# chalharu/rust-compression

Measured on AMD Instinct MI355X. Metric: BZip2 level-9 encode MB/s (input bytes, HBM-resident in and out: the kernels' rate; value_end_to_end is host buffer to host buffer at the C ABI), higher is better.
Workload: dtype u8/u32

## Files before the change

### rust-compression_amd/csrc/k_mtf.hip

```cpp
#include "bzgpu.h"
#include <cstdlib>

namespace bzgpu {

constexpr u32 kChunkWGs = (kMaxMtfChunks + 255) / 256;
constexpr u32 kMtfSmallAlpha = 96;

__device__ __forceinline__ u32 popc8(const u32 *b)
{
    u32 c = 0;
#pragma unroll
    for (int i = 0; i < 8; ++i) c += __popc(b[i]);
    return c;
}

__device__ __forceinline__ u32 block_excl_sum(u32 v, u32 *sh , u32 &total)
{
    const u32 l = lane_id(), w = threadIdx.x >> 6;
    const u32 inc = wave_incl_sum(v);
    if (l == 63) sh[w] = inc;
    __syncthreads();
    u32 carry = 0, tot = 0;
    for (u32 k = 0; k < kSortThreads / 64; ++k) {
        if (k < w) carry += sh[k];
        tot += sh[k];
    }
    total = tot;
    __syncthreads();
    return carry + inc - v;
}

constexpr u32 kMtfDense = 0x80000000u;
__device__ __forceinline__ bool mtf_collapsed(const MtfArgs &a, u32 lb) { return a.heads && !(a.hcount[lb] & kMtfDense); }
__device__ __forceinline__ u32 mtf_len(const MtfArgs &a, u32 lb) { return mtf_collapsed(a, lb) ? a.hcount[lb] : a.blocks[lb].n; }
__device__ __forceinline__ const u8 *mtf_seq(const MtfArgs &a, u32 lb) { return (mtf_collapsed(a, lb) ? a.H : a.L) + (size_t)lb * kSlot; }

__global__ __launch_bounds__(kSortThreads) void k_mtf_heads_mark(MtfArgs a)
{
    __shared__ u32 s_cnt[kSortThreads / 64];
    const u32 lb = blockIdx.y, tile = blockIdx.x;
    const u32 n = a.blocks[lb].n;
    if (n == 0u && tile == 0u && threadIdx.x == 0u) a.hcount[lb] = 0u;
    if (tile * kSortTile >= n) return;
    const u8 *L = a.L + (size_t)lb * kSlot;
    const u32 p0 = tile * kSortTile + threadIdx.x * 16u;
    const u32 valid = p0 < n ? ((n - p0) < 16u ? (n - p0) : 16u) : 0u;
    u32 hb = 0;
    if (valid) {
        const uint4 q = *reinterpret_cast<const uint4 *>(L + p0);
        const u32 prev = p0 ? (u32)L[p0 - 1u] : 0u;
        const u32 wv[4] = {q.x, q.y, q.z, q.w};
        u32 carry = prev;
#pragma unroll
        for (u32 w = 0; w < 4; ++w) {
            const u32 d = wv[w] ^ ((wv[w] << 8) | carry);
            carry = wv[w] >> 24;
#pragma unroll
            for (u32 k = 0; k < 4; ++k) hb |= ((d >> (8u * k)) & 0xFFu) ? (1u << (4u * w + k)) : 0u;
        }
        if (p0 == 0u) hb |= 1u;
        hb &= 0xFFFFu >> (16u - valid);
        a.headbits[(((size_t)lb * kSlot) >> 4) + (p0 >> 4)] = (u16)hb;
    }
    const u32 c = wave_sum((u32)__popc(hb));
    if (lane_id() == 0) s_cnt[threadIdx.x >> 6] = c;
    __syncthreads();
    if (threadIdx.x == 0) {
        u32 t = 0;
        for (u32 k = 0; k < kSortThreads / 64; ++k) t += s_cnt[k];
        a.tile_hcnt[lb * kTilesPerBlock + tile] = t;
    }
}

__global__ __launch_bounds__(kSortThreads) void k_mtf_heads_pack(MtfArgs a)
{
    __shared__ __attribute__((aligned(16))) u8 s_h[kSortTile + 16];
    __shared__ u32 s_su[kSortThreads / 64];
    __shared__ u32 s_pre[4];
    const u32 lb = blockIdx.y, tile = blockIdx.x;
    const u32 n = a.blocks[lb].n;
    if (tile * kSortTile >= n) return;
    const u8 *L = a.L + (size_t)lb * kSlot;
    const u32 p0 = tile * kSortTile + threadIdx.x * 16u;
    const bool valid = p0 < n;
    if (threadIdx.x < 128u) {
        static_assert(kTilesPerBlock <= 128, "two waves sum the tiles in front");
        const u32 ntiles = (n + kSortTile - 1u) / kSortTile;
        const u32 c = threadIdx.x < ntiles ? a.tile_hcnt[lb * kTilesPerBlock + threadIdx.x] : 0u;
        const u32 pre = wave_sum(threadIdx.x < tile ? c : 0u), all = wave_sum(c);
        if (lane_id() == 0) {
            s_pre[threadIdx.x >> 6] = pre;
            s_pre[2u + (threadIdx.x >> 6)] = all;
        }
    }
    __syncthreads();
    const u32 m = s_pre[2] + s_pre[3];
    if ((u64)m * 1000u > (u64)n * a.dense_permille) {
        if (tile == 0u && threadIdx.x == 0u) a.hcount[lb] = kMtfDense | m;
        return;
    }
    const u32 hb = valid ? (u32)a.headbits[(((size_t)lb * kSlot) >> 4) + (p0 >> 4)] : 0u;
    const uint4 q = valid ? *reinterpret_cast<const uint4 *>(L + p0) : make_uint4(0, 0, 0, 0);
    u32 total;
    const u32 excl = block_excl_sum((u32)__popc(hb), s_su, total);
    const u32 base = s_pre[0] + s_pre[1];
    const u32 al = base & 3u;
    {
        const u32 wv[4] = {q.x, q.y, q.z, q.w};
        u32 pos = al + excl;
#pragma unroll
        for (u32 k = 0; k < 16; ++k)
            if ((hb >> k) & 1u) s_h[pos++] = (u8)(wv[k >> 2] >> ((k & 3) * 8));
    }
    __syncthreads();
    u8 *dst = a.H + (size_t)lb * kSlot + (base - al);
    const u32 endb = al + total;
    for (u32 j = threadIdx.x; j * 4u < endb; j += kSortThreads) {
        if (j * 4u >= al && j * 4u + 4u <= endb) {
            reinterpret_cast<u32 *>(dst)[j] = reinterpret_cast<const u32 *>(s_h)[j];
        } else {
            for (u32 b = j * 4u; b < j * 4u + 4u; ++b)
                if (b >= al && b < endb) dst[b] = s_h[b];
        }
    }
    if (threadIdx.x == 0) {
        a.tile_hbase[lb * kTilesPerBlock + tile] = base;
        if (tile == 0u) a.hcount[lb] = m;
    }
}

__global__ __launch_bounds__(256) void k_mtf_summaries(MtfArgs a)
{
    __shared__ u32 s_seen[8 * 256];
    const u32 lb = blockIdx.y;
    const u32 n = mtf_len(a, lb);
    const u32 chunk = blockIdx.x * 256u + threadIdx.x;
    const u32 beg = chunk * kMtfChunk;
    if (beg >= n) return;
    const u32 end = (beg + kMtfChunk < n) ? beg + kMtfChunk : n;
    const u32 alpha = popc8(a.inuse_bits + lb * 8);
#pragma unroll
    for (int i = 0; i < 8; ++i) s_seen[i * 256 + threadIdx.x] = 0;
    const u8 *L = mtf_seq(a, lb);
    u8 *out = a.summ + ((size_t)lb * kMaxMtfChunks + chunk) * 256u;
    u32 cnt = 0;
    for (int v4 = (int)(kMtfChunk / 64u) - 1; v4 >= 0 && cnt < alpha; --v4) {
        if (beg + (u32)v4 * 64u >= end) continue;
        uint4 q4[4];
#pragma unroll
        for (int u = 0; u < 4; ++u) {
            const u32 pl = beg + (u32)v4 * 64u + (u32)u * 16u;
            q4[u] = (pl < end) ? *reinterpret_cast<const uint4 *>(L + pl) : make_uint4(0, 0, 0, 0);
        }
#pragma unroll
        for (int u = 3; u >= 0; --u) {
            const u32 p0 = beg + (u32)v4 * 64u + (u32)u * 16u;
            if (p0 >= end || cnt >= alpha) continue;
            const u32 wv[4] = {q4[u].x, q4[u].y, q4[u].z, q4[u].w};
#pragma unroll
            for (int k = 15; k >= 0; --k) {
                if (p0 + (u32)k < end) {
                    const u32 c = (wv[k >> 2] >> ((k & 3) * 8)) & 0xFFu;
                    const u32 bit = 1u << (c & 31u);
                    const u32 wd = s_seen[(c >> 5) * 256 + threadIdx.x];
                    if (!(wd & bit)) {
                        s_seen[(c >> 5) * 256 + threadIdx.x] = wd | bit;
                        out[cnt++] = (u8)c;
                    }
                }
            }
        }
    }
    a.summ_len[(size_t)lb * kMaxMtfChunks + chunk] = (u16)cnt;
}


constexpr u32 kMtfGroup = 32;
constexpr u32 kMtfGroups = (kMaxMtfChunks + kMtfGroup - 1) / kMtfGroup;

__device__ __forceinline__ u32 mtf_apply_report(u8 *s_list, u32 len, u32 m, u32 w, u8 *s_new, u8 *s_mark, u32 l)
{
    reinterpret_cast<u32 *>(s_mark)[l] = 0;
    __syncthreads();
#pragma unroll
    for (u32 k = 0; k < 4; ++k) {
        const u32 i = l * 4u + k;
        if (i < m) {
            const u8 v = (u8)(w >> (8u * k));
            s_mark[v] = 1;
            s_new[i] = v;
        }
    }
    __syncthreads();
    u32 keep[4], nk = 0;
    u8 ev[4];
#pragma unroll
    for (u32 k = 0; k < 4; ++k) {
        const u32 e = l * 4 + k;
        ev[k] = s_list[e];
        keep[k] = (e < len && !s_mark[ev[k]]) ? 1u : 0u;
        nk += keep[k];
    }
    const u32 inc = wave_incl_sum(nk);
    u32 pos = m + inc - nk;
#pragma unroll
    for (u32 k = 0; k < 4; ++k)
        if (keep[k]) s_new[pos++] = ev[k];
    const u32 kept = __shfl(inc, 63, 64);
    __syncthreads();
    reinterpret_cast<u32 *>(s_list)[l] = reinterpret_cast<u32 *>(s_new)[l];
    __syncthreads();
    return m + kept;
}

__global__ __launch_bounds__(64) void k_mtf_merge_groups(MtfArgs a)
{
    __shared__ u8 s_cur[256], s_new[256], s_mark[256];
    const u32 lb = blockIdx.y, l = threadIdx.x;
    const u32 n = mtf_len(a, lb);
    const u32 nchunks = (n + kMtfChunk - 1) / kMtfChunk;
    const u32 c0 = blockIdx.x * kMtfGroup;
    if (c0 + 2u > nchunks) return;
    const size_t rep0 = (size_t)lb * kMaxMtfChunks;
    const bool act = l * 4u < popc8(a.inuse_bits + lb * 8);
    u32 len = a.summ_len[rep0 + c0];
    reinterpret_cast<u32 *>(s_cur)[l] = act ? reinterpret_cast<const u32 *>(a.summ + (rep0 + c0) * 256u)[l] : 0u;
    __syncthreads();
    u32 c1 = c0 + kMtfGroup;
    if (c1 > nchunks - 1u) c1 = nchunks - 1u;
    u32 m_next = c0 + 1u < c1 ? (u32)a.summ_len[rep0 + c0 + 1u] : 0u;
    u32 w_next = (c0 + 1u < c1 && act) ? reinterpret_cast<const u32 *>(a.summ + (rep0 + c0 + 1u) * 256u)[l] : 0u;
    for (u32 c = c0 + 1u; c < c1; ++c) {
        const u32 m = m_next, w = w_next;
        if (c + 1u < c1) {
            m_next = a.summ_len[rep0 + c + 1u];
            w_next = act ? reinterpret_cast<const u32 *>(a.summ + (rep0 + c + 1u) * 256u)[l] : 0u;
        }
        len = mtf_apply_report(s_cur, len, m, w, s_new, s_mark, l);
        if (act) reinterpret_cast<u32 *>(a.summ + (rep0 + c) * 256u)[l] = reinterpret_cast<u32 *>(s_cur)[l];
        if (l == 0) a.summ_len[rep0 + c] = (u16)len;
    }
}

__global__ __launch_bounds__(64) void k_mtf_group_starts(MtfArgs a)
{
    __shared__ u8 s_state[256], s_new[256], s_mark[256];
    const u32 lb = blockIdx.x, l = threadIdx.x;
    const u32 n = mtf_len(a, lb);
    const u32 nchunks = (n + kMtfChunk - 1) / kMtfChunk;
    const u32 *bits = a.inuse_bits + lb * 8;
    {
        u32 before = 0;
        for (u32 q = 0; q < (l * 4u) / 32u; ++q) before += __popc(bits[q]);
        const u32 wd = bits[(l * 4u) >> 5];
        const u32 sh = (l * 4u) & 31u;
        before += __popc(wd & ((1u << sh) - 1u));
        reinterpret_cast<u32 *>(s_state)[l] = 0;
        __syncthreads();
        u32 pos = before;
        for (u32 k = 0; k < 4; ++k)
            if ((wd >> (sh + k)) & 1u) s_state[pos++] = (u8)(l * 4u + k);
    }
    __syncthreads();
    const u32 alpha = popc8(bits);
    const size_t rep0 = (size_t)lb * kMaxMtfChunks;
    const bool act = l * 4u < alpha;
    for (u32 c0 = 0; c0 < nchunks; c0 += kMtfGroup) {
        if (act) reinterpret_cast<u32 *>(a.init_state + (rep0 + c0) * 256u)[l] = reinterpret_cast<u32 *>(s_state)[l];
        if (c0 + 2u > nchunks) break;
        u32 e = c0 + kMtfGroup - 1u;
        if (e > nchunks - 2u) e = nchunks - 2u;
        const u32 m = a.summ_len[rep0 + e];
        const u32 w = act ? reinterpret_cast<const u32 *>(a.summ + (rep0 + e) * 256u)[l] : 0u;
        (void)mtf_apply_report(s_state, alpha, m, w, s_new, s_mark, l);
    }
}

__global__ __launch_bounds__(256) void k_mtf_chunk_starts(MtfArgs a)
{
    __shared__ u8 s_state[4][256], s_new[4][256], s_mark[4][256];
    const u32 lb = blockIdx.y, l = threadIdx.x & 63u, wv = threadIdx.x >> 6;
    const u32 n = mtf_len(a, lb);
    const u32 nchunks = (n + kMtfChunk - 1) / kMtfChunk;
    const u32 c0 = blockIdx.x * kMtfGroup;
    if (c0 + 1u >= nchunks) return;
    const u32 alpha = popc8(a.inuse_bits + lb * 8);
    const size_t rep0 = (size_t)lb * kMaxMtfChunks;
    const bool act = l * 4u < alpha;
    const u32 g32 = act ? reinterpret_cast<const u32 *>(a.init_state + (rep0 + c0) * 256u)[l] : 0u;
    for (u32 k = 0; k < kMtfGroup / 4u; ++k) {
        const u32 c = c0 + 1u + k * 4u + wv;
        const bool live = c < nchunks && c < c0 + kMtfGroup;
        reinterpret_cast<u32 *>(s_state[wv])[l] = g32;
        const u32 m = live ? (u32)a.summ_len[rep0 + c - 1u] : 0u;
        const u32 w = (live && act) ? reinterpret_cast<const u32 *>(a.summ + (rep0 + c - 1u) * 256u)[l] : 0u;
        (void)mtf_apply_report(s_state[wv], alpha, m, w, s_new[wv], s_mark[wv], l);
        if (live && act) reinterpret_cast<u32 *>(a.init_state + (rep0 + c) * 256u)[l] = reinterpret_cast<u32 *>(s_state[wv])[l];
    }
}


constexpr u32 kMtfSmallPairs = kMtfSmallAlpha / 2;
constexpr u32 kMtfSubBlocks = 16;
typedef short short2_t __attribute__((ext_vector_type(2)));
__device__ __forceinline__ short2_t as_short2(u32 v)
{
    short2_t r;
    __builtin_memcpy(&r, &v, 4);
    return r;
}
template <u32 PAIRS, u32 LANES, u32 ALPHA_LO, u32 SUB = 1>
__global__ __launch_bounds__(LANES) void k_mtf_ranks_small(MtfArgs a)
{
    constexpr u32 CL = LANES / SUB;
    __shared__ u32 s_last[PAIRS * CL];
    __shared__ u8 s_code[256];
    const u32 lb = blockIdx.y;
    const u32 n = mtf_len(a, lb);
    const u32 chunk0 = blockIdx.x * CL;
    const u32 sub = threadIdx.x % SUB;
    if (chunk0 * kMtfChunk >= n) return;
    const u32 *bits = a.inuse_bits + lb * 8;
    const u32 alpha = popc8(bits);
    if (alpha > 2u * PAIRS || alpha <= ALPHA_LO) return;
    for (u32 v = threadIdx.x; v < 256u; v += LANES) {
        u32 before = 0;
        for (u32 q = 0; q < (v >> 5); ++q) before += __popc(bits[q]);
        before += __popc(bits[v >> 5] & ((1u << (v & 31u)) - 1u));
        s_code[v] = (u8)before;
    }
    __syncthreads();
    const u32 chunk = chunk0 + threadIdx.x / SUB;
    const u32 beg = chunk * kMtfChunk;
    if (beg >= n) return;
    const u32 end = (beg + kMtfChunk < n) ? beg + kMtfChunk : n;
    const u32 npairs = (alpha + 1u) >> 1;
    u32 *my = s_last + threadIdx.x / SUB;
    constexpr u32 kPB = 32;
    static_assert(PAIRS % (2u * kPB) == 0 || PAIRS <= kMtfSmallPairs, "the compare loop takes the table two blocks at a time");
    const u32 npairs16 = ((npairs + 2u * kPB - 1u) / (2u * kPB) * (2u * kPB)) < PAIRS ? ((npairs + 2u * kPB - 1u) / (2u * kPB) * (2u * kPB)) : PAIRS;
    for (u32 q = sub; q < (SUB > 1 ? PAIRS : npairs16); q += SUB) my[q * CL] = 0x80008000u;
    if (SUB > 1) {
        __builtin_amdgcn_fence(__ATOMIC_ACQ_REL, "workgroup");
        __builtin_amdgcn_wave_barrier();
    }
    if (sub == 0) {
        const u8 *st = a.init_state + ((size_t)lb * kMaxMtfChunks + chunk) * 256u;
        for (u32 q = 0; q < alpha; ++q) {
            const u32 c = s_code[st[q]];
            const u32 t = (u32)(0xFFFFu - q) & 0xFFFFu;
            u32 wd = my[(c >> 1) * CL];
            wd = (c & 1u) ? ((wd & 0x0000FFFFu) | (t << 16)) : ((wd & 0xFFFF0000u) | t);
            my[(c >> 1) * CL] = wd;
        }
    }
    if (SUB > 1) {
        __builtin_amdgcn_fence(__ATOMIC_ACQ_REL, "workgroup");
        __builtin_amdgcn_wave_barrier();
    }
    const u8 *L = mtf_seq(a, lb);
    u8 *R8 = a.rank8 + (size_t)lb * kSlot;
    for (u32 v4 = 0; v4 < kMtfChunk / 64u; ++v4) {
        if (beg + v4 * 64u >= end) break;
        uint4 q4[4];
#pragma unroll
        for (u32 u = 0; u < 4; ++u) {
            const u32 pl = beg + v4 * 64u + u * 16u;
            q4[u] = (pl < end) ? *reinterpret_cast<const uint4 *>(L + pl) : make_uint4(0, 0, 0, 0);
        }
#pragma unroll
      for (u32 u = 0; u < 4; ++u) {
        const u32 v = v4 * 4u + u;
        const u32 p0 = beg + v * 16u;
        if (p0 >= end) break;
        const u32 wv[4] = {q4[u].x, q4[u].y, q4[u].z, q4[u].w};
        u32 ov[4] = {0, 0, 0, 0};
#pragma unroll
        for (u32 k = 0; k < 16; ++k) {
            u32 rank = 0;
            if (p0 + k < end) {
                const u32 c = s_code[(wv[k >> 2] >> ((k & 3) * 8)) & 0xFFu];
                const u32 wc = my[(c >> 1) * CL];
                const u32 lsu = (c & 1u) ? (wc >> 16) : (wc & 0xFFFFu);
                const short2_t ls2 = as_short2(lsu | (lsu << 16));
                short2_t acc = {0, 0};
              if (SUB == 1 && PAIRS > kMtfSmallPairs) {
                u32 ra[kPB], rb[kPB];
#pragma unroll
                for (u32 e = 0; e < kPB; ++e) ra[e] = my[e * CL];
                for (u32 q = 0; q < npairs16; q += 2u * kPB) {
#pragma unroll
                    for (u32 e = 0; e < kPB; ++e) rb[e] = my[(q + kPB + e) * CL];
#pragma unroll
                    for (u32 e = 0; e < kPB; ++e) acc -= __builtin_elementwise_sub_sat(ls2, as_short2(ra[e])) >> (short2_t){15, 15};
                    const u32 qn = (q + 2u * kPB < npairs16) ? q + 2u * kPB : 0u;
#pragma unroll
                    for (u32 e = 0; e < kPB; ++e) ra[e] = my[(qn + e) * CL];
#pragma unroll
                    for (u32 e = 0; e < kPB; ++e) acc -= __builtin_elementwise_sub_sat(ls2, as_short2(rb[e])) >> (short2_t){15, 15};
                }
              } else if (SUB > 1) {
                constexpr u32 PER = PAIRS / SUB;
                u32 ra[PER];
#pragma unroll
                for (u32 e = 0; e < PER; ++e) ra[e] = my[(sub * PER + e) * CL];
#pragma unroll
                for (u32 e = 0; e < PER; ++e) acc -= __builtin_elementwise_sub_sat(ls2, as_short2(ra[e])) >> (short2_t){15, 15};
              } else
                for (u32 q = 0; q < npairs; ++q) {
                    const short2_t wd = as_short2(my[q * CL]);
                    const short2_t neg = __builtin_elementwise_sub_sat(ls2, wd) >> (short2_t){15, 15};
                    acc -= neg;
                }
                rank = (u32)(int)acc.x + (u32)(int)acc.y;
                if (SUB > 1) {
#pragma unroll
                    for (u32 d = 1; d < SUB; d <<= 1) rank += (u32)__shfl_xor((int)rank, (int)d, 64);
                }
                const u32 t = (v * 16u + k) & 0xFFFFu;
                if (sub == 0) my[(c >> 1) * CL] = (c & 1u) ? ((wc & 0x0000FFFFu) | (t << 16)) : ((wc & 0xFFFF0000u) | t);
            }
            ov[k >> 2] |= rank << ((k & 3) * 8);
        }
        if (sub == 0) *reinterpret_cast<uint4 *>(R8 + p0) = make_uint4(ov[0], ov[1], ov[2], ov[3]);
      }
    }
}

struct ZSeg {
    u8 r[16];
    u32 valid;
    u32 p0;
    int next_nonzero;
};

__device__ __forceinline__ void zload(const MtfArgs &a, u32 lb, u32 n, u32 tile, ZSeg &s)
{
    const u8 *__restrict__ R8 = a.rank8 + (size_t)lb * kSlot;
    s.p0 = tile * kSortTile + threadIdx.x * 16u;
    s.valid = s.p0 < n ? ((n - s.p0) < 16u ? (n - s.p0) : 16u) : 0u;
    if (mtf_collapsed(a, lb)) {
        __shared__ __attribute__((aligned(16))) u8 s_hr[kSortTile + 32];
        __shared__ u32 s_hs[kSortThreads / 64];
        const u16 *hbits = a.headbits + (((size_t)lb * kSlot) >> 4);
        const u32 hb = s.valid ? (u32)hbits[s.p0 >> 4] : 0u;
        const u32 hbase = a.tile_hbase[lb * kTilesPerBlock + tile];
        const u32 m = a.hcount[lb];
        const u32 a0 = hbase & ~15u;
        {
            const u32 off = a0 + threadIdx.x * 16u;
            if (off < m) *reinterpret_cast<uint4 *>(s_hr + threadIdx.x * 16u) = *reinterpret_cast<const uint4 *>(R8 + off);
            if (threadIdx.x == 0 && a0 + kSortTile < m)
                *reinterpret_cast<uint4 *>(s_hr + kSortTile) = *reinterpret_cast<const uint4 *>(R8 + a0 + kSortTile);
        }
        u32 total;
        u32 pos = (hbase - a0) + block_excl_sum((u32)__popc(hb), s_hs, total);
#pragma unroll
        for (int k = 0; k < 16; ++k) {
            const bool h = (hb >> k) & 1u;
            s.r[k] = h ? s_hr[pos] : (u8)0;
            pos += h ? 1u : 0u;
        }
        const u32 nx = s.p0 + s.valid;
        s.next_nonzero = (s.valid == 0u || nx >= n) ? 1 : (int)(hbits[nx >> 4] & 1u);
        return;
    }
    if (s.valid) {
        const uint4 q = *reinterpret_cast<const uint4 *>(R8 + s.p0);
        const u32 wv[4] = {q.x, q.y, q.z, q.w};
#pragma unroll
        for (int k = 0; k < 16; ++k) s.r[k] = (u8)(wv[k >> 2] >> ((k & 3) * 8));
        const u32 nx = s.p0 + s.valid;
        s.next_nonzero = (nx >= n) ? 1 : (R8[nx] != 0);
    } else {
        s.next_nonzero = 1;
    }
}

__device__ __forceinline__ int block_excl_max_int(int v, int *sh )
{
    const u32 l = lane_id(), w = threadIdx.x >> 6;
    const int inc = wave_incl_max32(v);
    if (l == 63) sh[w] = inc;
    __syncthreads();
    int carry = -1;
    for (u32 k = 0; k < w; ++k) carry = sh[k] > carry ? sh[k] : carry;
    const int prev = __shfl_up(inc, 1, 64);
    const int ex = (l == 0) ? -1 : prev;
    __syncthreads();
    return ex > carry ? ex : carry;
}

__global__ __launch_bounds__(kSortThreads) void k_zle_last(MtfArgs a)
{
    __shared__ int s_last;
    const u32 lb = blockIdx.y, tile = blockIdx.x;
    const u32 n = a.blocks[lb].n;
    if (tile * kSortTile >= n) return;
    if (threadIdx.x == 0) s_last = -1;
    __syncthreads();
    ZSeg s;
    zload(a, lb, n, tile, s);
    int last = -1;
#pragma unroll
    for (u32 k = 0; k < 16; ++k)
        if (k < s.valid && s.r[k]) last = (int)(s.p0 + k);
#pragma unroll
    for (u32 dd = 32; dd >= 1; dd >>= 1) {
        const int o = __shfl_xor(last, dd, 64);
        last = o > last ? o : last;
    }
    if (lane_id() == 0 && last >= 0) atomicMax(&s_last, last);
    __syncthreads();
    if (threadIdx.x == 0) a.ztile_last[lb * kTilesPerBlock + tile] = s_last;
}

__device__ __forceinline__ u32 run_digits(u32 z) { return 31u - (u32)__clz(z + 1u); }

template <bool WRITE>
__global__ __launch_bounds__(kSortThreads) void k_zle_emit(MtfArgs a)
{
    __shared__ int s_mi[16];
    __shared__ u32 s_su[16];
    __shared__ u32 s_freq[kMaxAlpha + 2];
    __shared__ int s_carry;
    __shared__ u32 s_base;
    __shared__ u16 s_out[WRITE ? kSortTile + 64 : 1];
    const u32 lb = blockIdx.y, tile = blockIdx.x;
    const u32 n = a.blocks[lb].n;
    if (tile * kSortTile >= n) return;
    if (threadIdx.x == 0) {
        int c = -1;
        for (int t = (int)tile - 1; t >= 0 && c < 0; --t) c = a.ztile_last[lb * kTilesPerBlock + t];
        s_carry = c;
        if (WRITE) {
            u32 b = 0;
            for (u32 t = 0; t < tile; ++t) b += a.ztile_cnt[lb * kTilesPerBlock + t];
            s_base = b;
        }
    }
    if (WRITE)
        for (u32 i = threadIdx.x; i < kMaxAlpha + 2; i += kSortThreads) s_freq[i] = 0;
    __syncthreads();
    ZSeg s;
    zload(a, lb, n, tile, s);
    int last = -1;
#pragma unroll
    for (u32 k = 0; k < 16; ++k)
        if (k < s.valid && s.r[k]) last = (int)(s.p0 + k);
    int lnz = block_excl_max_int(last, s_mi);
    lnz = lnz > s_carry ? lnz : s_carry;
    u32 cnt = 0;
    {
        int ln = lnz;
#pragma unroll
        for (u32 k = 0; k < 16; ++k) {
            if (k < s.valid) {
                const u32 p = s.p0 + k;
                if (s.r[k]) {
                    ln = (int)p;
                    cnt += 1;
                } else {
                    const bool run_end = (k + 1 < s.valid) ? (s.r[(k + 1) & 15] != 0) : (s.next_nonzero != 0);
                    if (run_end) cnt += run_digits((u32)((int)p - ln));
                }
            }
        }
    }
    u32 total;
    u32 off = block_excl_sum(cnt, s_su, total);
    if (!WRITE) {
        if (threadIdx.x == 0) a.ztile_cnt[lb * kTilesPerBlock + tile] = total;
        return;
    }
    u16 *out = s_out + off;
    u32 hot0 = 0, hot1 = 0, hot2 = 0, hot3 = 0;
    {
        int ln = lnz;
#pragma unroll
        for (u32 k = 0; k < 16; ++k) {
            if (k < s.valid) {
                const u32 p = s.p0 + k;
                if (s.r[k]) {
                    ln = (int)p;
                    const u32 sym = (u32)s.r[k] + 1u;
                    *out++ = (u16)sym;
                    if (sym == 2u) ++hot2;
                    else if (sym == 3u) ++hot3;
                    else atomicAdd(&s_freq[sym], 1u);
                } else {
                    const bool run_end = (k + 1 < s.valid) ? (s.r[(k + 1) & 15] != 0) : (s.next_nonzero != 0);
                    if (run_end) {
                        u32 zc = (u32)((int)p - ln) + 1u;
                        while (zc > 1u) {
                            const u32 run = zc & 1u;
                            *out++ = (u16)run;
                            hot0 += run ^ 1u;
                            hot1 += run;
                            zc >>= 1;
                        }
                    }
                }
            }
        }
    }
    hot0 = wave_sum(hot0);
    hot1 = wave_sum(hot1);
    hot2 = wave_sum(hot2);
    hot3 = wave_sum(hot3);
    if ((threadIdx.x & 63u) == 0) {
        if (hot0) atomicAdd(&s_freq[0], hot0);
        if (hot1) atomicAdd(&s_freq[1], hot1);
        if (hot2) atomicAdd(&s_freq[2], hot2);
        if (hot3) atomicAdd(&s_freq[3], hot3);
    }
    __syncthreads();
    {
        u16 *dst = a.mtf + (size_t)lb * kMtfStride + s_base;
        for (u32 i = threadIdx.x; i < total; i += kSortThreads) dst[i] = s_out[i];
    }
    const bool last_tile = (tile + 1) * kSortTile >= n;
    if (last_tile && threadIdx.x == 0) {
        const u32 alpha_in = popc8(a.inuse_bits + lb * 8);
        const u32 eob = alpha_in + 1u;
        a.mtf[(size_t)lb * kMtfStride + s_base + total] = (u16)eob;
        atomicAdd(&s_freq[eob], 1u);
        a.out[lb].mtf_count = s_base + total + 1u;
        a.out[lb].in_use_count = alpha_in;
    }
    __syncthreads();
    for (u32 i = threadIdx.x; i < kMaxAlpha; i += kSortThreads)
        if (s_freq[i]) atomicAdd(&a.mtf_freq[(size_t)lb * kMaxAlpha + i], s_freq[i]);
}

__global__ __launch_bounds__(kSortThreads) void k_zle_fused(MtfArgs a)
{
    __shared__ int s_mi[16];
    __shared__ u32 s_su[16];
    __shared__ u32 s_freq[kMaxAlpha + 2];
    __shared__ int s_carry;
    __shared__ u32 s_base, s_ticket;
    __shared__ u16 s_out[kSortTile + 64];
    const u32 xcd = (u32)__builtin_amdgcn_s_getreg(20 | (3 << 11)) & 7u;
    const u32 my_tiles = a.tiles * ((a.nb + 7u - xcd) / 8u);
    if (threadIdx.x == 0) s_ticket = atomicAdd(&a.ztick[xcd], 1u);
    __syncthreads();
    const u32 slot = s_ticket;
    if (slot >= my_tiles) return;
    const u32 b8 = slot / a.tiles;
    const u32 tile = slot - b8 * a.tiles;
    const u32 lb = b8 * 8u + xcd;
    const u32 n = a.blocks[lb].n;
    if (tile * kSortTile >= n) return;
    for (u32 i = threadIdx.x; i < kMaxAlpha + 2; i += kSortThreads) s_freq[i] = 0;
    ZSeg s;
    zload(a, lb, n, tile, s);
    int last = -1;
#pragma unroll
    for (u32 k = 0; k < 16; ++k)
        if (k < s.valid && s.r[k]) last = (int)(s.p0 + k);
    int lnz = block_excl_max_int(last, s_mi);
    u32 *mystate = a.zstate + ((size_t)lb * kTilesPerBlock + tile) * 4u;
    u32 w_last = 0;
    if (threadIdx.x == 0) {
        int tl = -1;
        for (u32 k = 0; k < kSortThreads / 64; ++k) tl = s_mi[k] > tl ? s_mi[k] : tl;
        const u32 vl = tl >= 0 ? (u32)tl : kLbValMask;
        st_sc1_x4(mystate, make_uint4((tile ? kLbAgg : kLbIncl) | vl, 0u, 0u, 0u));
        int c = -1;
        if (tile) {
            u32 spins = 0;
            for (u32 p = tile; p > 0 && c < 0;) {
                --p;
                const u32 *src = a.zstate + ((size_t)lb * kTilesPerBlock + p) * 4u;
                uint4 v = ld_sc1_x4(src);
                while ((v.x & kLbFlagMask) == 0u) {
                    if (lb_give_up(spins, a.ztick + 8, kLbSpinMax >> 3)) {
                        atomicExch(a.ztick + 8, 1u);
                        v = make_uint4(kLbIncl, 0u, 0u, 0u);
                        break;
                    }
                    __builtin_amdgcn_s_sleep(2);
                    v = ld_sc1_x4(src);
                }
                const u32 x = v.x & kLbValMask;
                if (x != kLbValMask) c = (int)x;
                else if ((v.x & kLbFlagMask) == kLbIncl) break;
            }
        }
        w_last = kLbIncl | (tl >= 0 ? (u32)tl : (c >= 0 ? (u32)c : kLbValMask));
        if (tile) st_sc1_x4(mystate, make_uint4(w_last, 0u, 0u, 0u));
        s_carry = c;
    }
    __syncthreads();
    lnz = lnz > s_carry ? lnz : s_carry;
    u32 cnt = 0;
    {
        int ln = lnz;
#pragma unroll
        for (u32 k = 0; k < 16; ++k) {
            if (k < s.valid) {
                const u32 p = s.p0 + k;
                if (s.r[k]) {
                    ln = (int)p;
                    cnt += 1;
                } else {
                    const bool run_end = (k + 1 < s.valid) ? (s.r[(k + 1) & 15] != 0) : (s.next_nonzero != 0);
                    if (run_end) cnt += run_digits((u32)((int)p - ln));
                }
            }
        }
    }
    u32 total;
    const u32 off = block_excl_sum(cnt, s_su, total);
    if (threadIdx.x == 0) st_sc1_x4(mystate, make_uint4(w_last, (tile ? kLbAgg : kLbIncl) | total, 0u, 0u));
    u16 *out = s_out + off;
    u32 hot0 = 0, hot1 = 0, hot2 = 0, hot3 = 0;
    {
        int ln = lnz;
#pragma unroll
        for (u32 k = 0; k < 16; ++k) {
            if (k < s.valid) {
                const u32 p = s.p0 + k;
                if (s.r[k]) {
                    ln = (int)p;
                    const u32 sym = (u32)s.r[k] + 1u;
                    *out++ = (u16)sym;
                    if (sym == 2u) ++hot2;
                    else if (sym == 3u) ++hot3;
                    else atomicAdd(&s_freq[sym], 1u);
                } else {
                    const bool run_end = (k + 1 < s.valid) ? (s.r[(k + 1) & 15] != 0) : (s.next_nonzero != 0);
                    if (run_end) {
                        u32 zc = (u32)((int)p - ln) + 1u;
                        while (zc > 1u) {
                            const u32 run = zc & 1u;
                            *out++ = (u16)run;
                            hot0 += run ^ 1u;
                            hot1 += run;
                            zc >>= 1;
                        }
                    }
                }
            }
        }
    }
    hot0 = wave_sum(hot0);
    hot1 = wave_sum(hot1);
    hot2 = wave_sum(hot2);
    hot3 = wave_sum(hot3);
    if ((threadIdx.x & 63u) == 0) {
        if (hot0) atomicAdd(&s_freq[0], hot0);
        if (hot1) atomicAdd(&s_freq[1], hot1);
        if (hot2) atomicAdd(&s_freq[2], hot2);
        if (hot3) atomicAdd(&s_freq[3], hot3);
    }
    if (threadIdx.x == 0) {
        u32 base = 0;
        if (tile) {
            u32 spins = 0;
            for (u32 p = tile; p > 0;) {
                --p;
                const u32 *src = a.zstate + ((size_t)lb * kTilesPerBlock + p) * 4u;
                uint4 v = ld_sc1_x4(src);
                while ((v.y & kLbFlagMask) == 0u) {
                    if (lb_give_up(spins, a.ztick + 8, kLbSpinMax >> 3)) {
                        atomicExch(a.ztick + 8, 1u);
                        v = make_uint4(0u, kLbIncl, 0u, 0u);
                        break;
                    }
                    __builtin_amdgcn_s_sleep(2);
                    v = ld_sc1_x4(src);
                }
                base += v.y & kLbValMask;
                if ((v.y & kLbFlagMask) == kLbIncl) break;
            }
            st_sc1_x4(mystate, make_uint4(w_last, kLbIncl | ((base + total) & kLbValMask), 0u, 0u));
        }
        s_base = base;
    }
    __syncthreads();
    {
        u16 *dst = a.mtf + (size_t)lb * kMtfStride + s_base;
        for (u32 i = threadIdx.x; i < total; i += kSortThreads) dst[i] = s_out[i];
    }
    const bool last_tile = (tile + 1) * kSortTile >= n;
    if (last_tile && threadIdx.x == 0) {
        const u32 alpha_in = popc8(a.inuse_bits + lb * 8);
        const u32 eob = alpha_in + 1u;
        a.mtf[(size_t)lb * kMtfStride + s_base + total] = (u16)eob;
        atomicAdd(&s_freq[eob], 1u);
        a.out[lb].mtf_count = s_base + total + 1u;
        a.out[lb].in_use_count = alpha_in;
    }
    __syncthreads();
    for (u32 i = threadIdx.x; i < kMaxAlpha; i += kSortThreads)
        if (s_freq[i]) atomicAdd(&a.mtf_freq[(size_t)lb * kMaxAlpha + i], s_freq[i]);
}

void launch_mtf(hipStream_t st, const MtfArgs &a, KernelProf *prof, u64 total_n)
{
    (void)hipMemsetAsync(a.mtf_freq, 0, (size_t)a.nb * kMaxAlpha * sizeof(u32), st);
    if (a.heads) {
        const int pi = prof ? prof->begin(st, KID_MTF_HEADS, 2u * total_n + total_n / 2u) : -1;
        hipLaunchKernelGGL(k_mtf_heads_mark, dim3(a.tiles, a.nb), dim3(kSortThreads), 0, st, a);
        hipLaunchKernelGGL(k_mtf_heads_pack, dim3(a.tiles, a.nb), dim3(kSortThreads), 0, st, a);
        if (prof) prof->end(st, pi);
    }
    hipLaunchKernelGGL(k_mtf_summaries, dim3(kChunkWGs, a.nb), dim3(256), 0, st, a);
    hipLaunchKernelGGL(k_mtf_merge_groups, dim3(kMtfGroups, a.nb), dim3(64), 0, st, a);
    hipLaunchKernelGGL(k_mtf_group_starts, dim3(a.nb), dim3(64), 0, st, a);
    hipLaunchKernelGGL(k_mtf_chunk_starts, dim3(kMtfGroups, a.nb), dim3(256), 0, st, a);
    if (a.nb <= kMtfSubBlocks) {
        hipLaunchKernelGGL((k_mtf_ranks_small<kMtfSmallPairs, 256, 0, 8>), dim3((kMaxMtfChunks + 31) / 32, a.nb), dim3(256), 0, st, a);
        hipLaunchKernelGGL((k_mtf_ranks_small<128, 128, kMtfSmallAlpha, 8>), dim3((kMaxMtfChunks + 15) / 16, a.nb), dim3(128), 0, st, a);
    } else {
        hipLaunchKernelGGL((k_mtf_ranks_small<kMtfSmallPairs, 256, 0>), dim3(kChunkWGs, a.nb), dim3(256), 0, st, a);
        hipLaunchKernelGGL((k_mtf_ranks_small<128, 128, kMtfSmallAlpha>), dim3((kMaxMtfChunks + 127) / 128, a.nb), dim3(128), 0, st, a);
    }
    if (a.fused_zle) {
        (void)hipMemsetAsync(a.zstate, 0, (size_t)a.nb * kTilesPerBlock * 16, st);
        (void)hipMemsetAsync(a.ztick, 0, 64, st);
        hipLaunchKernelGGL(k_zle_fused, dim3(a.tiles, xcd_grid_y(a.nb)), dim3(kSortThreads), 0, st, a);
        return;
    }
    const dim3 grid(a.tiles, a.nb);
    hipLaunchKernelGGL(k_zle_last, grid, dim3(kSortThreads), 0, st, a);
    hipLaunchKernelGGL((k_zle_emit<false>), grid, dim3(kSortThreads), 0, st, a);
    hipLaunchKernelGGL((k_zle_emit<true>), grid, dim3(kSortThreads), 0, st, a);
}

}
```

Before: 15310.

## Represent ZLE segments as nonzero bitmasks and iterate events with ffs

Replaces the per-thread 16-byte rank array with a 16-bit nonzero mask plus packed words, using SWAR byte tests and alignbyte extraction instead of per-byte unpacking and shared-memory gathers. Run ends are found with bit operations, and count and write loops walk only the set event bits via ffs rather than a fully unrolled 16-step branchy loop. The four hot-symbol counters are packed into one register as byte fields. The loops become data-dependent with divergence across lanes, and the packed 8-bit counters could overflow if one thread emits 256 or more of a single symbol.

```diff
diff --git a/rust-compression_amd/csrc/k_mtf.hip b/rust-compression_amd/csrc/k_mtf.hip
--- a/rust-compression_amd/csrc/k_mtf.hip
+++ b/rust-compression_amd/csrc/k_mtf.hip
@@ -428,18 +428,29 @@
 }
 
 struct ZSeg {
-    u8 r[16];
+    u32 nz;
+    u32 q[4];
+    u32 j0;
+    bool by_head;
     u32 valid;
     u32 p0;
     int next_nonzero;
 };
 
+__device__ __forceinline__ u32 nonzero_bytes(u32 v)
+{
+    const u32 t = ((((v & 0x7F7F7F7Fu) + 0x7F7F7F7Fu) | v) & 0x80808080u) >> 7;
+    return (t * 0x01020408u) >> 24;
+}
+
 __device__ __forceinline__ void zload(const MtfArgs &a, u32 lb, u32 n, u32 tile, ZSeg &s)
 {
     const u8 *__restrict__ R8 = a.rank8 + (size_t)lb * kSlot;
     s.p0 = tile * kSortTile + threadIdx.x * 16u;
     s.valid = s.p0 < n ? ((n - s.p0) < 16u ? (n - s.p0) : 16u) : 0u;
-    if (mtf_collapsed(a, lb)) {
+    s.j0 = 0;
+    s.by_head = mtf_collapsed(a, lb);
+    if (s.by_head) {
         __shared__ __attribute__((aligned(16))) u8 s_hr[kSortTile + 32];
         __shared__ u32 s_hs[kSortThreads / 64];
         const u16 *hbits = a.headbits + (((size_t)lb * kSlot) >> 4);
@@ -454,12 +465,18 @@
                 *reinterpret_cast<uint4 *>(s_hr + kSortTile) = *reinterpret_cast<const uint4 *>(R8 + a0 + kSortTile);
         }
         u32 total;
-        u32 pos = (hbase - a0) + block_excl_sum((u32)__popc(hb), s_hs, total);
-#pragma unroll
-        for (int k = 0; k < 16; ++k) {
-            const bool h = (hb >> k) & 1u;
-            s.r[k] = h ? s_hr[pos] : (u8)0;
-            pos += h ? 1u : 0u;
+        const u32 pos = (hbase - a0) + block_excl_sum((u32)__popc(hb), s_hs, total);
+        const u32 *hw = reinterpret_cast<const u32 *>(s_hr) + (pos >> 2);
+        const u32 w0 = hw[0], w1 = hw[1], w2 = hw[2], w3 = hw[3], w4 = hw[4];
+        const u32 sh = pos & 3u;
+        s.q[0] = __builtin_amdgcn_alignbyte(w1, w0, sh);
+        s.q[1] = __builtin_amdgcn_alignbyte(w2, w1, sh);
+        s.q[2] = __builtin_amdgcn_alignbyte(w3, w2, sh);
+        s.q[3] = __builtin_amdgcn_alignbyte(w4, w3, sh);
+        s.nz = hb;
+        if (s.p0 == 0u && (s.q[0] & 0xFFu) == 0u) {
+            s.nz = hb & ~1u;
+            s.j0 = 1;
         }
         const u32 nx = s.p0 + s.valid;
         s.next_nonzero = (s.valid == 0u || nx >= n) ? 1 : (int)(hbits[nx >> 4] & 1u);
@@ -467,13 +484,66 @@
     }
     if (s.valid) {
         const uint4 q = *reinterpret_cast<const uint4 *>(R8 + s.p0);
-        const u32 wv[4] = {q.x, q.y, q.z, q.w};
-#pragma unroll
-        for (int k = 0; k < 16; ++k) s.r[k] = (u8)(wv[k >> 2] >> ((k & 3) * 8));
+        s.q[0] = q.x, s.q[1] = q.y, s.q[2] = q.z, s.q[3] = q.w;
+        s.nz = (nonzero_bytes(q.x) | (nonzero_bytes(q.y) << 4) | (nonzero_bytes(q.z) << 8) | (nonzero_bytes(q.w) << 12)) &
+               (0xFFFFu >> (16u - s.valid));
         const u32 nx = s.p0 + s.valid;
         s.next_nonzero = (nx >= n) ? 1 : (R8[nx] != 0);
     } else {
+        s.q[0] = s.q[1] = s.q[2] = s.q[3] = 0;
+        s.nz = 0;
         s.next_nonzero = 1;
+    }
+}
+
+__device__ __forceinline__ int zseg_last(const ZSeg &s) { return s.nz ? (int)(s.p0 + 31u - (u32)__clz(s.nz)) : -1; }
+
+__device__ __forceinline__ u32 zseg_run_ends(const ZSeg &s)
+{
+    if (s.valid == 0u) return 0u;
+    return ~s.nz & ((s.nz >> 1) | ((u32)s.next_nonzero << (s.valid - 1u))) & (0xFFFFu >> (16u - s.valid));
+}
+
+__device__ __forceinline__ u32 run_digits(u32 z) { return 31u - (u32)__clz(z + 1u); }
+
+__device__ __forceinline__ u32 zseg_count(const ZSeg &s, u32 re, int lnz)
+{
+    u32 cnt = (u32)__popc(s.nz);
+    while (re) {
+        const u32 k = (u32)__ffs((int)re) - 1u;
+        re &= re - 1u;
+        const u32 below = s.nz & ((1u << k) - 1u);
+        const int ln = below ? (int)(s.p0 + 31u - (u32)__clz(below)) : lnz;
+        cnt += run_digits((u32)((int)(s.p0 + k) - ln));
+    }
+    return cnt;
+}
+
+__device__ __forceinline__ void zseg_write(const ZSeg &s, u32 re, int lnz, u16 *out, u32 *s_freq, u32 &hot)
+{
+    u32 ev = s.nz | re;
+    int ln = lnz;
+    u32 j = s.j0;
+    const u64 qlo = ((u64)s.q[1] << 32) | s.q[0], qhi = ((u64)s.q[3] << 32) | s.q[2];
+    while (ev) {
+        const u32 k = (u32)__ffs((int)ev) - 1u;
+        ev &= ev - 1u;
+        const bool is_nz = (s.nz >> k) & 1u;
+        const int p = (int)(s.p0 + k);
+        const u32 idx = s.by_head ? j : k;
+        const u32 rank = (u32)((idx < 8u ? qlo : qhi) >> ((idx & 7u) * 8u)) & 0xFFu;
+        u32 zc = is_nz ? 1u : (u32)(p - ln) + 1u;
+        u32 sym = is_nz ? rank + 1u : (zc & 1u);
+        j += is_nz ? 1u : 0u;
+        ln = is_nz ? p : ln;
+        for (;;) {
+            *out++ = (u16)sym;
+            if (sym < 4u) hot += 1u << (sym * 8u);
+            else atomicAdd(&s_freq[sym], 1u);
+            zc >>= 1;
+            if (zc <= 1u) break;
+            sym = zc & 1u;
+        }
     }
 }
 
@@ -501,10 +571,7 @@
     __syncthreads();
     ZSeg s;
     zload(a, lb, n, tile, s);
-    int last = -1;
-#pragma unroll
-    for (u32 k = 0; k < 16; ++k)
-        if (k < s.valid && s.r[k]) last = (int)(s.p0 + k);
+    int last = zseg_last(s);
 #pragma unroll
     for (u32 dd = 32; dd >= 1; dd >>= 1) {
         const int o = __shfl_xor(last, dd, 64);
@@ -514,8 +581,6 @@
     __syncthreads();
     if (threadIdx.x == 0) a.ztile_last[lb * kTilesPerBlock + tile] = s_last;
 }
-
-__device__ __forceinline__ u32 run_digits(u32 z) { return 31u - (u32)__clz(z + 1u); }
 
 template <bool WRITE>
 __global__ __launch_bounds__(kSortThreads) void k_zle_emit(MtfArgs a)
@@ -544,29 +609,11 @@
     __syncthreads();
     ZSeg s;
     zload(a, lb, n, tile, s);
-    int last = -1;
-#pragma unroll
-    for (u32 k = 0; k < 16; ++k)
-        if (k < s.valid && s.r[k]) last = (int)(s.p0 + k);
+    int last = zseg_last(s);
     int lnz = block_excl_max_int(last, s_mi);
     lnz = lnz > s_carry ? lnz : s_carry;
-    u32 cnt = 0;
-    {
-        int ln = lnz;
-#pragma unroll
-        for (u32 k = 0; k < 16; ++k) {
-            if (k < s.valid) {
-                const u32 p = s.p0 + k;
-                if (s.r[k]) {
-                    ln = (int)p;
-                    cnt += 1;
-                } else {
-                    const bool run_end = (k + 1 < s.valid) ? (s.r[(k + 1) & 15] != 0) : (s.next_nonzero != 0);
-                    if (run_end) cnt += run_digits((u32)((int)p - ln));
-                }
-            }
-        }
-    }
+    const u32 re = zseg_run_ends(s);
+    const u32 cnt = zseg_count(s, re, lnz);
     u32 total;
     u32 off = block_excl_sum(cnt, s_su, total);
     if (!WRITE) {
@@ -574,40 +621,12 @@
         return;
     }
     u16 *out = s_out + off;
-    u32 hot0 = 0, hot1 = 0, hot2 = 0, hot3 = 0;
-    {
-        int ln = lnz;
-#pragma unroll
-        for (u32 k = 0; k < 16; ++k) {
-            if (k < s.valid) {
-                const u32 p = s.p0 + k;
-                if (s.r[k]) {
-                    ln = (int)p;
-                    const u32 sym = (u32)s.r[k] + 1u;
-                    *out++ = (u16)sym;
-                    if (sym == 2u) ++hot2;
-                    else if (sym == 3u) ++hot3;
-                    else atomicAdd(&s_freq[sym], 1u);
-                } else {
-                    const bool run_end = (k + 1 < s.valid) ? (s.r[(k + 1) & 15] != 0) : (s.next_nonzero != 0);
-                    if (run_end) {
-                        u32 zc = (u32)((int)p - ln) + 1u;
-                        while (zc > 1u) {
-                            const u32 run = zc & 1u;
-                            *out++ = (u16)run;
-                            hot0 += run ^ 1u;
-                            hot1 += run;
-                            zc >>= 1;
-                        }
-                    }
-                }
-            }
-        }
-    }
-    hot0 = wave_sum(hot0);
-    hot1 = wave_sum(hot1);
-    hot2 = wave_sum(hot2);
-    hot3 = wave_sum(hot3);
+    u32 hot = 0;
+    zseg_write(s, re, lnz, out, s_freq, hot);
+    const u32 hot0 = wave_sum(hot & 0xFFu);
+    const u32 hot1 = wave_sum((hot >> 8) & 0xFFu);
+    const u32 hot2 = wave_sum((hot >> 16) & 0xFFu);
+    const u32 hot3 = wave_sum(hot >> 24);
     if ((threadIdx.x & 63u) == 0) {
         if (hot0) atomicAdd(&s_freq[0], hot0);
         if (hot1) atomicAdd(&s_freq[1], hot1);
@@ -655,10 +674,7 @@
     for (u32 i = threadIdx.x; i < kMaxAlpha + 2; i += kSortThreads) s_freq[i] = 0;
     ZSeg s;
     zload(a, lb, n, tile, s);
-    int last = -1;
-#pragma unroll
-    for (u32 k = 0; k < 16; ++k)
-        if (k < s.valid && s.r[k]) last = (int)(s.p0 + k);
+    int last = zseg_last(s);
     int lnz = block_excl_max_int(last, s_mi);
     u32 *mystate = a.zstate + ((size_t)lb * kTilesPerBlock + tile) * 4u;
     u32 w_last = 0;
@@ -694,61 +710,18 @@
     }
     __syncthreads();
     lnz = lnz > s_carry ? lnz : s_carry;
-    u32 cnt = 0;
-    {
-        int ln = lnz;
-#pragma unroll
-        for (u32 k = 0; k < 16; ++k) {
-            if (k < s.valid) {
-                const u32 p = s.p0 + k;
-                if (s.r[k]) {
-                    ln = (int)p;
-                    cnt += 1;
-                } else {
-                    const bool run_end = (k + 1 < s.valid) ? (s.r[(k + 1) & 15] != 0) : (s.next_nonzero != 0);
-                    if (run_end) cnt += run_digits((u32)((int)p - ln));
-                }
-            }
-        }
-    }
+    const u32 re = zseg_run_ends(s);
+    const u32 cnt = zseg_count(s, re, lnz);
     u32 total;
     const u32 off = block_excl_sum(cnt, s_su, total);
     if (threadIdx.x == 0) st_sc1_x4(mystate, make_uint4(w_last, (tile ? kLbAgg : kLbIncl) | total, 0u, 0u));
     u16 *out = s_out + off;
-    u32 hot0 = 0, hot1 = 0, hot2 = 0, hot3 = 0;
-    {
-        int ln = lnz;
-#pragma unroll
-        for (u32 k = 0; k < 16; ++k) {
-            if (k < s.valid) {
-                const u32 p = s.p0 + k;
-                if (s.r[k]) {
-                    ln = (int)p;
-                    const u32 sym = (u32)s.r[k] + 1u;
-                    *out++ = (u16)sym;
-                    if (sym == 2u) ++hot2;
-                    else if (sym == 3u) ++hot3;
-                    else atomicAdd(&s_freq[sym], 1u);
-                } else {
-                    const bool run_end = (k + 1 < s.valid) ? (s.r[(k + 1) & 15] != 0) : (s.next_nonzero != 0);
-                    if (run_end) {
-                        u32 zc = (u32)((int)p - ln) + 1u;
-                        while (zc > 1u) {
-                            const u32 run = zc & 1u;
-                            *out++ = (u16)run;
-                            hot0 += run ^ 1u;
-                            hot1 += run;
-                            zc >>= 1;
-                        }
-                    }
-                }
-            }
-        }
-    }
-    hot0 = wave_sum(hot0);
-    hot1 = wave_sum(hot1);
-    hot2 = wave_sum(hot2);
-    hot3 = wave_sum(hot3);
+    u32 hot = 0;
+    zseg_write(s, re, lnz, out, s_freq, hot);
+    const u32 hot0 = wave_sum(hot & 0xFFu);
+    const u32 hot1 = wave_sum((hot >> 8) & 0xFFu);
+    const u32 hot2 = wave_sum((hot >> 16) & 0xFFu);
+    const u32 hot3 = wave_sum(hot >> 24);
     if ((threadIdx.x & 63u) == 0) {
         if (hot0) atomicAdd(&s_freq[0], hot0);
         if (hot1) atomicAdd(&s_freq[1], hot1);
```

Measured after the change: 15450 (median of 6 runs). Within noise of the previous version (+0.9%).
